# feinanshan/TDNet

Hardware: AMD Instinct MI355X
Metric: frames/sec (td4-psp18, 1024x2048, full-resolution logits) (higher is better)
Workload: dtype f32; 1 GPU; td4-psp18, 1024x2048 Cityscapes-shaped synthetic stream, 3-frame feature cache, 1 clip per GPU; parallelism=clip-parallel x1, RCCL weight broadcast only, target_fps_per_gpu=30

## Files before the change

### tdnet_amd/csrc/td_launch.h

```cpp
#pragma once
#include "td_weights.h"

#ifdef TDNET_TIMING_PROBES
static int probe_skip() {
    static const int m = [] {
        const char* e = getenv("TDNET_PROBE_SKIP");
        const int v = e ? atoi(e) : 0;
        if (v) fprintf(stderr, "tdnet: TDNET_PROBE_SKIP=%d -- pieces of the frame are NOT computed, every result of this process is garbage (timing probe build)\n", v);
        return v;
    }();
    return m;
}
#else
static constexpr int probe_skip() { return 0; }
#endif
static void prof_begin(tdnet* n, int family, int dominant, double flops, hipStream_t s) {
    if (!n || !n->prof) return;
    if (n->nrec == n->recs.size()) {
        ProfRec r;
        hipEventCreate(&r.e0); hipEventCreate(&r.e1);
        n->recs.push_back(r);
    }
    ProfRec& r = n->recs[n->nrec];
    r.family = family; r.dominant = dominant; r.flops = flops;
    hipEventRecord(r.e0, s);
}
static void prof_end(tdnet* n, hipStream_t s) {
    if (!n || !n->prof) return;
    hipEventRecord(n->recs[n->nrec].e1, s);
    n->nrec++;
}

struct LnFuse { const float *mean, *rstd, *g, *b; };

struct WinoChunk { int ny = 1, cy = 0, nx = 1, cx = 0; };

template <int VW>
static void launch_wino4_c(bool out_side, const WinoArgs& wa, hipStream_t s) {
    if (out_side) TD_LAUNCH((k_wino4_out_c<VW>), dim3(wino_chunk_grid(wa.Tc, wa.Cout, VW)), dim3(256), 0, s, wa);
    else TD_LAUNCH((k_wino4_in_c<VW>), dim3(wino_chunk_grid(wa.Tc, wa.C, VW)), dim3(256), 0, s, wa);
}

static ConvArgs conv_args(const ConvLayer& L, const float* in, int H, int W, const float* resid, float* out) {
    const int Ho = out_size(H, L.KS, L.stride, L.dil, L.pad), Wo = out_size(W, L.KS, L.stride, L.dil, L.pad);
    return ConvArgs{in, L.d_wp, L.d_bias, resid, out, H, W, L.Cin, Wo, L.Cout, L.CoutPad, L.stride, L.dil, L.pad, Ho * Wo, L.nsteps, L.act, 0, 1};
}
static GemmArgs gemm_args(const ConvLayer& L, const float* a, int M, int nbatch, const float* bias, const float* resid, float* out, int act) {
    GemmArgs ga;
    ga.a = a; ga.wp = L.d_wp; ga.bias = bias; ga.resid = resid; ga.out = out;
    ga.M = M; ga.N = L.Cout; ga.NPad = L.CoutPad; ga.K = L.Cin; ga.nbatch = nbatch; ga.act = act; ga.tiles_m = ga.tiles_n = 0; ga.MP = M;
    return ga;
}
static void launch_gemm(const ConvLayer& L, const GemmArgs& ga, int b3_grid, hipStream_t s) {
    const int forced_grid = L.pers > 1 ? L.pers : 0;
    switch (L.gemm) {
    case GK_B3: gemm_b3_launch(ga, forced_grid ? forced_grid : b3_grid, s); break;
    case GK_DMA: gemm_dma_launch(ga, forced_grid, s); break;
    case GK_PERSISTENT: gemm_launch(ga, L.tile, forced_grid, s); break;
    case GK_CONV:
        conv_launch(ConvArgs{ga.a, ga.wp, ga.bias, ga.resid, ga.out, 1, ga.M, ga.K, ga.M, ga.N, ga.NPad, 1, 1, 0, ga.M, L.nsteps, ga.act, 0, ga.nbatch}, L.tile, 1, false, s);
        break;
    }
}

static int run_wino(tdnet* n, const ConvLayer& L, const float* in, int H, int W, const float* resid, float* out, hipStream_t s,
                    const LnFuse* lnf, const WinoChunk& ck, float* V, float* Mb, const ClsArgs* cls = nullptr) {
    const int TY = wino_tiles_1d(H, L.dil, L.wino), TX = wino_tiles_1d(W, L.dil, L.wino);
    const long T = (long)L.dil * L.dil * TY * TX;
    const bool chunked = ck.ny != 1 || ck.nx != 1;
    if (chunked && (!L.vw || L.dil % ck.ny || L.dil % ck.nx)) return td_fail("internal: this conv cannot run in chunks");
    const long Tc = (long)(L.dil / ck.ny) * (L.dil / ck.nx) * TY * TX;
    const int nb = (L.wino + 2) * (L.wino + 2);
    bool own = false;
    if (!V) {
        own = n == nullptr || n->wino_v_floats < (size_t)nb * Tc * L.Cin || n->wino_m_floats < (size_t)nb * Tc * L.Cout;
        if (own) {
            if (n) { n->failed = true; return td_fail("internal: Winograd workspace too small"); }
            if (dev_alloc(&V, (size_t)nb * Tc * L.Cin) || dev_alloc(&Mb, (size_t)nb * Tc * L.Cout)) return -1;
        } else { V = n->wino_v; Mb = n->wino_m; }
    }
    WinoArgs wa;
    wa.in = in; wa.V = V; wa.Mb = Mb; wa.bias = L.d_bias; wa.resid = resid; wa.out = out;
    wa.H = H; wa.W = W; wa.C = L.Cin; wa.Cout = L.Cout; wa.dil = L.dil; wa.TY = TY; wa.TX = TX; wa.T = (int)T; wa.act = L.act; wa.TP = (int)Tc;
    wa.ln_mean = lnf ? lnf->mean : nullptr; wa.ln_rstd = lnf ? lnf->rstd : nullptr; wa.ln_g = lnf ? lnf->g : nullptr; wa.ln_b = lnf ? lnf->b : nullptr;
    wa.Tc = (int)Tc; wa.ny = ck.ny; wa.cy = ck.cy; wa.nx = ck.nx; wa.cx = ck.cx;
    auto transform = [&](bool out_side) {
        if (n && (probe_skip() & 1)) return;
        prof_begin(n, 2, false, 0, s);
        const int C = out_side ? L.Cout : L.Cin;
        if (out_side && cls) {
            const unsigned grid = (unsigned)((Tc + 3) / 4);
            if (L.Cout == 128) TD_LAUNCH((k_wino4_out_cls<2>), dim3(grid), dim3(256), wino_out_cls_lds(128, cls->NC), s, wa, *cls);
            else TD_LAUNCH((k_wino4_out_cls<1>), dim3(grid), dim3(256), wino_out_cls_lds(64, cls->NC), s, wa, *cls);
        } else
        if (L.vw == 1) launch_wino4_c<1>(out_side, wa, s);
        else if (L.vw == 2 && C % 2 == 0) launch_wino4_c<2>(out_side, wa, s);
        else if (L.vw == 4 && C % 4 == 0) launch_wino4_c<4>(out_side, wa, s);
        else if (L.vw) launch_wino4_c<1>(out_side, wa, s);
        else if (out_side) TD_LAUNCH(k_wino4_out, dim3(td_grid_for(T * (L.Cout / 4), 256, 256 * 16)), dim3(256), 0, s, wa);
        else TD_LAUNCH(k_wino4_in, dim3(td_grid_for(T * (L.Cin / 4), 256, 256 * 16)), dim3(256), 0, s, wa);
        prof_end(n, s);
    };
    transform(false);
    prof_begin(n, 0, 2, 2.0 * nb * Tc * (double)L.Cin * L.Cout, s);
    if (!(n && (probe_skip() & 8))) launch_gemm(L, gemm_args(L, V, (int)Tc, nb, L.d_zero, nullptr, Mb, 0), chunked ? 320 : 0, s);
    prof_end(n, s);
    transform(true);
    if (own) { TD_HIP(hipStreamSynchronize(s)); hipFree(V); hipFree(Mb); }
    return 0;
}

static void launch_conv_dma_forms(const ConvLayer& L, const ConvArgs& a, hipStream_t s) {
    int rh = L.rh;
    bool done = false;
    const bool is192 = rh == CD_192_P || rh == CD_192_N;
    if (rh == CD_128_N || rh == CD_192_N) {
        done = !L.rowimg_off && conv_launch_dma3n(a, rh, L.KS, L.out16, s);
        if (!done) rh = is192 ? CD_192_P : CD_128_P;
    }
    if (!done && (rh == CD_128_P || rh == CD_192_P)) {
        done = !L.rowimg_off && conv_launch_dma3p(a, rh, L.KS, L.out16, s);
        if (!done) rh = is192 ? CD_192 : CD_128_8W;
    }
    if (!done && (L.rowimg_off || !conv_launch_dma3(a, rh, L.KS, L.out16, s))) conv_launch_dma(a, rh, L.KS, L.out16, s);
}

static int run_conv(tdnet* n, const ConvLayer& L, const float* in, int H, int W, const float* resid, float* out, hipStream_t s,
                    int* Ho_out = nullptr, int* Wo_out = nullptr, const LnFuse* lnf = nullptr, const ClsArgs* cls = nullptr) {
    if (lnf && !L.wino) return td_fail("internal: LayerNorm fusion needs a Winograd input transform");
    if (cls && (!L.wino || L.chunks > 1 || resid)) return td_fail("internal: the classifier rides in a whole Winograd conv's output transform");
    const int Ho = out_size(H, L.KS, L.stride, L.dil, L.pad), Wo = out_size(W, L.KS, L.stride, L.dil, L.pad);
    if (L.wino) {
        if (Ho_out) *Ho_out = H;
        if (Wo_out) *Wo_out = W;
        if (L.chunks > 1 && (!n || !n->ws_ready)) {
            for (int c = 0; c < L.chunks; ++c) {
                WinoChunk ck; ck.ny = L.chunks; ck.cy = c;
                TD_TRY(run_wino(n, L, in, H, W, resid, out, s, lnf, ck, nullptr, nullptr));
            }
            return 0;
        }
        return run_wino(n, L, in, H, W, resid, out, s, lnf, WinoChunk(), nullptr, nullptr, cls);
    }
    const ConvArgs a = conv_args(L, in, H, W, resid, out);
    prof_begin(n, 0, (((L.tile == CT_128x128 || L.tile == CT_128x128_DEEP || L.rh) && L.KS == 3 && !L.stem) ? 1 : 0) | ((L.h16() && L.in16 && L.KS == 3 && !L.stem) ? 4 : 0), L.flops_per_pixel() * a.M, s);
    switch (L.route) {
    case CR_STEM_H: conv_launch_stem_h(a, L.out16, s); break;
    case CR_CONV_DMA: launch_conv_dma_forms(L, a, s); break;
    case CR_CONV_H: conv_launch_h(a, L.tile, L.KS, L.in16, L.out16, s); break;
    case CR_ADIRECT_B3: conv_launch_adirect_b3(a, L.KS, 0, s); break;
    case CR_GEMM1X1: launch_gemm(L, gemm_args(L, in, a.M, 1, L.d_bias, resid, out, L.act), 0, s); break;
    case CR_ADIRECT_ROWS:
    case CR_ADIRECT_ROWS_B3: {
        ConvArgs r = a;
        r.H = stem_rows_hp(H); r.W = stem_rows_wp(W); r.Cin = 3; r.pad = 0;
        if (L.route == CR_ADIRECT_ROWS_B3) conv_launch_adirect_b3(r, L.KS, 2, s);
        else conv_launch_adirect(r, L.KS, 2, s);
        break;
    }
    case CR_ADIRECT: conv_launch_adirect(a, L.KS, L.stem ? 1 : 0, s); break;
    case CR_IGEMM: conv_launch(a, L.tile, L.KS, L.stem, s); break;
    case CR_WINO: break;
    }
    prof_end(n, s);
    if (Ho_out) *Ho_out = Ho;
    if (Wo_out) *Wo_out = Wo;
    return 0;
}

struct ConvCall { const ConvLayer* L; const float* in; int H, W; float* out; };
static int run_conv_group(tdnet* n, const ConvCall* c, int ng, hipStream_t s, int* Ho_out = nullptr, int* Wo_out = nullptr) {
    bool same = n && (n->opts.fusion & TDNET_FUSION_CONV_GROUPS) && ng >= 2 && ng <= 3;
    for (int g = 0; same && g < ng; ++g) {
        const ConvLayer& L = *c[g].L;
        const ConvLayer& L0 = *c[0].L;
        same = L.route == CR_CONV_H && L.in16 == L.out16 && L.in16 == L0.in16 && (g == 0 ? (L.KS == 1 || L.KS == 3) : L.KS == 1) &&
               conv_tile_dims(L.tile).BM == conv_tile_dims(L0.tile).BM && conv_tile_dims(L.tile).BN == conv_tile_dims(L0.tile).BN;
    }
    if (!same) {
        for (int g = 0; g < ng; ++g) TD_TRY(run_conv(n, *c[g].L, c[g].in, c[g].H, c[g].W, nullptr, c[g].out, s, g == 0 ? Ho_out : nullptr, g == 0 ? Wo_out : nullptr));
        return 0;
    }
    ConvArgs a[3];
// ... 99 lines not shown
```

### tdnet_amd/csrc/td_wino.h

```cpp
#pragma once
#include "td_conv.h"

#include <vector>

struct WinoArgs {
    const float* in;
    float* V;
    const float* Mb;
    const float* bias;
    const float* resid;
    float* out;
    int H, W, C, Cout, dil, TY, TX, T, act;
    int TP;
    const float* ln_mean; const float* ln_rstd; const float* ln_g; const float* ln_b;
    int Tc, ny, cy, nx, cx;
};
struct WinoBufs { TdBuf in, g, b, resid, out; };
TD_DEV WinoBufs td_wino_bufs(const WinoArgs& p) {
    WinoBufs w;
    const unsigned pix = (unsigned)p.H * (unsigned)p.W;
    w.in = td_make_buf(p.in, pix * (unsigned)p.C * 4u);
    w.g = td_make_buf(p.ln_g, p.ln_mean ? pix * 4u : 0u);
    w.b = td_make_buf(p.ln_b, p.ln_mean ? pix * 4u : 0u);
    w.resid = td_make_buf(p.resid, p.resid ? pix * (unsigned)p.Cout * 4u : 0u);
    w.out = td_make_buf(p.out, pix * (unsigned)p.Cout * 4u);
    return w;
}
TD_DEV f32x4 td_wino_ld(const WinoArgs& p, const WinoBufs& w, int y, int x, int cv, const f32x4& m4, const f32x4& r4) {
    const bool ok = (unsigned)y < (unsigned)p.H && (unsigned)x < (unsigned)p.W;
    const unsigned pix = (unsigned)y * (unsigned)p.W + (unsigned)x;
    f32x4 z = td_buf_ld4(w.in, ok ? (pix * (unsigned)p.C + (unsigned)cv * 4u) * 4u : TD_BUF_OOB, 0u);
    if (p.ln_mean) {
        const float g = td_buf_ld1(w.g, ok ? pix * 4u : TD_BUF_OOB, 0u), b = td_buf_ld1(w.b, ok ? pix * 4u : TD_BUF_OOB, 0u);
        z = (z - m4) * r4 * g + b;
    }
    return z;
}

TD_DEV void td_wino4_bt(const f32x4 (&d)[6], f32x4 (&t)[6]) {
    const f32x4 a = d[4] - 4.f * d[2], b = d[3] - 4.f * d[1], c = d[4] - d[2], e = 2.f * (d[3] - d[1]);
    t[0] = 4.f * d[0] - 5.f * d[2] + d[4];
    t[1] = a + b;
    t[2] = a - b;
    t[3] = c + e;
    t[4] = c - e;
    t[5] = 4.f * d[1] - 5.f * d[3] + d[5];
}
TD_DEV void td_wino4_at(const f32x4 (&m)[6], f32x4 (&y)[4]) {
    const f32x4 p = m[1] + m[2], q = m[1] - m[2], r = m[3] + m[4], s = m[3] - m[4];
    y[0] = m[0] + p + r;
    y[1] = q + 2.f * s;
    y[2] = p + 4.f * r;
    y[3] = q + 8.f * s + m[5];
}

TD_KERNEL void TD_LAUNCH_BOUNDS(256, 2) k_wino4_in(WinoArgs p) {
    const int CV = p.C >> 2;
    const WinoBufs wb = td_wino_bufs(p);
    const long total = (long)p.T * CV;
    for (long i = (long)blockIdx.x * blockDim.x + threadIdx.x; i < total; i += (long)gridDim.x * blockDim.x) {
        const int cv = (int)(i % CV);
        int t = (int)(i / CV);
        const int tx = t % p.TX; t /= p.TX;
        const int ty = t % p.TY; t /= p.TY;
        const int px = t % p.dil, py = t / p.dil;
        f32x4 tm[6][6];
        f32x4 m4 = {0.f, 0.f, 0.f, 0.f}, r4 = m4;
        if (p.ln_mean) { m4 = td_ld4(p.ln_mean + cv * 4); r4 = td_ld4(p.ln_rstd + cv * 4); }
#pragma unroll
        for (int c = 0; c < 6; ++c) {
            const int x = px + p.dil * (4 * tx - 1 + c);
            f32x4 d[6], col[6];
#pragma unroll
            for (int r = 0; r < 6; ++r) d[r] = td_wino_ld(p, wb, py + p.dil * (4 * ty - 1 + r), x, cv, m4, r4);
            td_wino4_bt(d, col);
#pragma unroll
            for (int r = 0; r < 6; ++r) tm[r][c] = col[r];
        }
        const size_t tile = (size_t)(i / CV);
#pragma unroll
        for (int r = 0; r < 6; ++r) {
            f32x4 v[6];
            td_wino4_bt(tm[r], v);
#pragma unroll
            for (int c = 0; c < 6; ++c) td_st4(p.V + ((size_t)(r * 6 + c) * p.TP + tile) * p.C + cv * 4, v[c]);
        }
    }
}

TD_KERNEL void TD_LAUNCH_BOUNDS(256, 2) k_wino4_out(WinoArgs p) {
    const int CV = p.Cout >> 2;
    const WinoBufs wb = td_wino_bufs(p);
    const float slope = td_act_slope(p.act);
    const long total = (long)p.T * CV;
    for (long i = (long)blockIdx.x * blockDim.x + threadIdx.x; i < total; i += (long)gridDim.x * blockDim.x) {
        const int cv = (int)(i % CV);
        const size_t tile = (size_t)(i / CV);
        int t = (int)tile;
        const int tx = t % p.TX; t /= p.TX;
        const int ty = t % p.TY; t /= p.TY;
        const int px = t % p.dil, py = t / p.dil;
        unsigned offy[4], offx[4];
        bool oky[4], okx[4];
#pragma unroll
        for (int r = 0; r < 4; ++r) {
            const int y = py + p.dil * (4 * ty + r), x = px + p.dil * (4 * tx + r);
            oky[r] = y < p.H; okx[r] = x < p.W;
            offy[r] = (unsigned)y * (unsigned)p.W * (unsigned)p.Cout * 4u;
            offx[r] = ((unsigned)x * (unsigned)p.Cout + (unsigned)cv * 4u) * 4u;
        }
        f32x4 rs[4][4];
#pragma unroll
        for (int r = 0; r < 4; ++r)
#pragma unroll
            for (int c = 0; c < 4; ++c) rs[r][c] = td_buf_ld4(wb.resid, (oky[r] && okx[c]) ? offy[r] + offx[c] : TD_BUF_OOB, 0u);
        f32x4 sm[4][6];
#pragma unroll
        for (int c = 0; c < 6; ++c) {
            f32x4 m[6], col[4];
#pragma unroll
            for (int r = 0; r < 6; ++r) m[r] = td_ld4(p.Mb + ((size_t)(r * 6 + c) * p.TP + tile) * p.Cout + cv * 4);
            td_wino4_at(m, col);
#pragma unroll
            for (int r = 0; r < 4; ++r) sm[r][c] = col[r];
        }
        const f32x4 b = td_ld4(p.bias + cv * 4);
#pragma unroll
        for (int r = 0; r < 4; ++r) {
            f32x4 o4[4];
            td_wino4_at(sm[r], o4);
#pragma unroll
            for (int c = 0; c < 4; ++c) {
                f32x4 o = o4[c] + b;
                o = o + rs[r][c];
#pragma unroll
                for (int e = 0; e < 4; ++e) o[e] = td_activate(o[e], slope);
                td_buf_st4(wb.out, (oky[r] && okx[c]) ? offy[r] + offx[c] : TD_BUF_OOB, o);
            }
        }
    }
}


template <int VW> struct WinoVec;
template <> struct WinoVec<1> {
    typedef float T;
    TD_DEV_MEMBER T ld(TdBuf b, unsigned v, unsigned s) { return td_buf_ld1(b, v, s); }
    TD_DEV_MEMBER void st(TdBuf b, unsigned v, unsigned s, T x) { td_buf_st1(b, v, s, x); }
    TD_DEV_MEMBER T act(T x, float slope) { return td_activate(x, slope); }
};
template <> struct WinoVec<2> {
    typedef f32x2 T;
    TD_DEV_MEMBER T ld(TdBuf b, unsigned v, unsigned s) { return td_buf_ld2(b, v, s); }
    TD_DEV_MEMBER void st(TdBuf b, unsigned v, unsigned s, T x) { td_buf_st2(b, v, s, x); }
    TD_DEV_MEMBER T act(T x, float slope) { x[0] = td_activate(x[0], slope); x[1] = td_activate(x[1], slope); return x; }
};
template <> struct WinoVec<4> {
    typedef f32x4 T;
    TD_DEV_MEMBER T ld(TdBuf b, unsigned v, unsigned s) { return td_buf_ld4(b, v == TD_BUF_OOB ? v : v + s, 0u); }
    TD_DEV_MEMBER void st(TdBuf b, unsigned v, unsigned s, T x) { td_buf_st4(b, v == TD_BUF_OOB ? v : v + s, x); }
    TD_DEV_MEMBER T act(T x, float slope) {
#pragma unroll
        for (int e = 0; e < 4; ++e) x[e] = td_activate(x[e], slope);
        return x;
    }
};
template <typename T>
TD_DEV void td_wino4_bt_t(const T (&d)[6], T (&t)[6]) {
    const T a = d[4] - 4.f * d[2], b = d[3] - 4.f * d[1], c = d[4] - d[2], e = 2.f * (d[3] - d[1]);
    t[0] = 4.f * d[0] - 5.f * d[2] + d[4];
    t[1] = a + b;
    t[2] = a - b;
    t[3] = c + e;
    t[4] = c - e;
    t[5] = 4.f * d[1] - 5.f * d[3] + d[5];
}
template <typename T>
TD_DEV void td_wino4_at_t(const T (&m)[6], T (&y)[4]) {
    const T p = m[1] + m[2], q = m[1] - m[2], r = m[3] + m[4], s = m[3] - m[4];
    y[0] = m[0] + p + r;
    y[1] = q + 2.f * s;
    y[2] = p + 4.f * r;
    y[3] = q + 8.f * s + m[5];
}
struct WinoTile { int tl, sl, py, px, ty, tx; };
TD_DEV WinoTile td_wino_unit_tile(const WinoArgs& p, int slices, int wv) {
    WinoTile w;
    w.tl = wv / slices; w.sl = wv - w.tl * slices;
    int t = w.tl;
    w.tx = t % p.TX; t /= p.TX;
    w.ty = t % p.TY; t /= p.TY;
    const int pw = p.dil / p.nx;
    w.px = p.nx * (t % pw) + p.cx;
    w.py = p.ny * (t / pw) + p.cy;
    return w;
}

template <int VW, typename Mid>
TD_DEV void td_wino4_in_unit(const WinoArgs& p, int wv, Mid&& mid) {
    typedef WinoVec<VW> X;
    typedef typename X::T T;
    const int slices = (p.C + 64 * VW - 1) / (64 * VW);
    const WinoTile w = td_wino_unit_tile(p, slices, wv);
    const WinoBufs wb = td_wino_bufs(p);
    const int c0 = (w.sl * 64 + (int)(threadIdx.x & 63)) * VW;
    const unsigned coff = c0 < p.C ? (unsigned)c0 * 4u : TD_BUF_OOB;
    T m4 = T(0.f), r4 = T(0.f);
    if (p.ln_mean) {
        const TdBuf mb = td_make_buf(p.ln_mean, (unsigned)p.C * 4u), rb = td_make_buf(p.ln_rstd, (unsigned)p.C * 4u);
        m4 = X::ld(mb, coff, 0u); r4 = X::ld(rb, coff, 0u);
    }
    T dd[6][6];
#pragma unroll
    for (int c = 0; c < 6; ++c) {
        const int x = w.px + p.dil * (4 * w.tx - 1 + c);
#pragma unroll
        for (int r = 0; r < 6; ++r) {
            const int y = w.py + p.dil * (4 * w.ty - 1 + r);
            const bool ok = (unsigned)y < (unsigned)p.H && (unsigned)x < (unsigned)p.W;
            const unsigned pix = (unsigned)y * (unsigned)p.W + (unsigned)x;
            T z = X::ld(wb.in, ok ? coff : TD_BUF_OOB, ok ? pix * (unsigned)p.C * 4u : 0u);
            if (p.ln_mean) {
                const float g = td_buf_ld1(wb.g, ok ? 0u : TD_BUF_OOB, ok ? pix * 4u : 0u), b = td_buf_ld1(wb.b, ok ? 0u : TD_BUF_OOB, ok ? pix * 4u : 0u);
                z = (z - m4) * r4 * g + b;
            }
            dd[c][r] = z;
        }
    }
    mid();
    T tm[6][6];
#pragma unroll
    for (int c = 0; c < 6; ++c) {
        T col[6];
        td_wino4_bt_t(dd[c], col);
#pragma unroll
        for (int r = 0; r < 6; ++r) tm[r][c] = col[r];
    }
    mid();
    const unsigned plane = (unsigned)p.TP * (unsigned)p.C * 4u;
    const TdBuf vb = td_make_buf(p.V, 36u * plane);
    const unsigned voff = (unsigned)w.tl * (unsigned)p.C * 4u;
#pragma unroll
    for (int r = 0; r < 6; ++r) {
        T v[6];
        td_wino4_bt_t(tm[r], v);
#pragma unroll
        for (int c = 0; c < 6; ++c) X::st(vb, coff, (unsigned)(r * 6 + c) * plane + voff, v[c]);
    }
}

template <int VW, typename Mid>
TD_DEV void td_wino4_out_unit(const WinoArgs& p, int wv, Mid&& mid) {
    typedef WinoVec<VW> X;
    typedef typename X::T T;
    const int slices = (p.Cout + 64 * VW - 1) / (64 * VW);
    const WinoTile w = td_wino_unit_tile(p, slices, wv);
    const WinoBufs wb = td_wino_bufs(p);
    const float slope = td_act_slope(p.act);
    const int c0 = (w.sl * 64 + (int)(threadIdx.x & 63)) * VW;
    const unsigned coff = c0 < p.Cout ? (unsigned)c0 * 4u : TD_BUF_OOB;
    unsigned offy[4], offx[4];
    bool oky[4], okx[4];
#pragma unroll
    for (int r = 0; r < 4; ++r) {
        const int y = w.py + p.dil * (4 * w.ty + r), x = w.px + p.dil * (4 * w.tx + r);
        oky[r] = y < p.H; okx[r] = x < p.W;
        offy[r] = (unsigned)y * (unsigned)p.W * (unsigned)p.Cout * 4u;
        offx[r] = (unsigned)x * (unsigned)p.Cout * 4u;
    }
    T rs[4][4];
#pragma unroll
    for (int r = 0; r < 4; ++r)
#pragma unroll
        for (int c = 0; c < 4; ++c) {
            const bool ok = oky[r] && okx[c];
            rs[r][c] = X::ld(wb.resid, ok ? coff : TD_BUF_OOB, ok ? offy[r] + offx[c] : 0u);
        }
    const unsigned plane = (unsigned)p.TP * (unsigned)p.Cout * 4u;
    const TdBuf mb = td_make_buf(p.Mb, 36u * plane);
    const unsigned moff = (unsigned)w.tl * (unsigned)p.Cout * 4u;
    T mm[6][6];
#pragma unroll
    for (int c = 0; c < 6; ++c)
#pragma unroll
        for (int r = 0; r < 6; ++r) mm[c][r] = X::ld(mb, coff, (unsigned)(r * 6 + c) * plane + moff);
    const TdBuf bbuf = td_make_buf(p.bias, (unsigned)p.Cout * 4u);
    const T b = X::ld(bbuf, coff, 0u);
    mid();
    T sm[4][6];
#pragma unroll
    for (int c = 0; c < 6; ++c) {
        T col[4];
        td_wino4_at_t(mm[c], col);
#pragma unroll
        for (int r = 0; r < 4; ++r) sm[r][c] = col[r];
    }
    mid();
#pragma unroll
    for (int r = 0; r < 4; ++r) {
        T o4[4];
        td_wino4_at_t(sm[r], o4);
#pragma unroll
        for (int c = 0; c < 4; ++c) {
            const bool ok = oky[r] && okx[c];
            T o = o4[c] + b;
            o = o + rs[r][c];
            X::st(wb.out, ok ? coff : TD_BUF_OOB, ok ? offy[r] + offx[c] : 0u, X::act(o, slope));
        }
    }
}

template <int VW>
TD_KERNEL void TD_LAUNCH_BOUNDS(256, VW == 4 ? 2 : 4) k_wino4_in_c(WinoArgs p) {
    const int slices = (p.C + 64 * VW - 1) / (64 * VW);
    const int wv = TD_UNIFORM((int)((blockIdx.x * blockDim.x + threadIdx.x) >> 6));
    if (wv >= p.Tc * slices) return;
    td_wino4_in_unit<VW>(p, wv, []() {});
}
template <int VW>
TD_KERNEL void TD_LAUNCH_BOUNDS(256, VW == 4 ? 2 : 4) k_wino4_out_c(WinoArgs p) {
    const int slices = (p.Cout + 64 * VW - 1) / (64 * VW);
    const int wv = TD_UNIFORM((int)((blockIdx.x * blockDim.x + threadIdx.x) >> 6));
    if (wv >= p.Tc * slices) return;
    td_wino4_out_unit<VW>(p, wv, []() {});
}
struct ClsArgs { const float* w; const float* b; float* out; int NC; };
template <int VW>
TD_KERNEL void TD_LAUNCH_BOUNDS(256, 2) k_wino4_out_cls(WinoArgs p, ClsArgs c) {
    typedef WinoVec<VW> X;
    typedef typename X::T T;
    constexpr int C = 64 * VW, ROW = C + 4;
    TD_DYN_LDS(smem);
    float* ws = reinterpret_cast<float*>(smem);
    float* ys = ws + c.NC * C + (threadIdx.x >> 6) * (16 * ROW);
    for (int i = threadIdx.x; i < c.NC * C; i += blockDim.x) ws[i] = c.w[i];
    __syncthreads();
    const int wv = TD_UNIFORM((int)((blockIdx.x * blockDim.x + threadIdx.x) >> 6));
    if (wv >= p.Tc) return;
    const int lane = threadIdx.x & 63;
    const WinoTile w = td_wino_unit_tile(p, 1, wv);
    const float slope = td_act_slope(p.act);
    const unsigned coff = (unsigned)(lane * VW) * 4u;
    const unsigned plane = (unsigned)p.TP * (unsigned)C * 4u;
    const TdBuf mb = td_make_buf(p.Mb, 36u * plane);
    const unsigned moff = (unsigned)w.tl * (unsigned)C * 4u;
    T mm[6][6];
#pragma unroll
    for (int cc = 0; cc < 6; ++cc)
#pragma unroll
        for (int r = 0; r < 6; ++r) mm[cc][r] = X::ld(mb, coff, (unsigned)(r * 6 + cc) * plane + moff);
    const TdBuf bbuf = td_make_buf(p.bias, (unsigned)C * 4u);
    const T b = X::ld(bbuf, coff, 0u);
    T sm[4][6];
#pragma unroll
    for (int cc = 0; cc < 6; ++cc) {
        T col[4];
        td_wino4_at_t(mm[cc], col);
#pragma unroll
        for (int r = 0; r < 4; ++r) sm[r][cc] = col[r];
    }
#pragma unroll
    for (int r = 0; r < 4; ++r) {
        T o4[4];
        td_wino4_at_t(sm[r], o4);
#pragma unroll
        for (int cc = 0; cc < 4; ++cc) {
            T o = o4[cc] + b;
            o = o + T(0.f);
            o = X::act(o, slope);
            float* dst = ys + (r * 4 + cc) * ROW + lane * VW;
            if constexpr (VW == 1) dst[0] = o;
            else { dst[0] = o[0]; dst[1] = o[1]; }
        }
    }
    td_wave_sync();
    const int CQ = C >> 2;
    for (int idx = lane; idx < 16 * c.NC; idx += 64) {
        const int px = idx & 15, k = idx >> 4;
        const float* yr = ys + px * ROW;
        const float* wr = ws + k * C;
        float s[4];
#pragma unroll
        for (int qd = 0; qd < 4; ++qd) {
            float a = 0.f;
            for (int ch = 0; ch < CQ; ch += 4) {
                const f32x4 v = td_ld4(yr + qd * CQ + ch), u = td_ld4(wr + qd * CQ + ch);
                a = fmaf(v[0], u[0], a); a = fmaf(v[1], u[1], a); a = fmaf(v[2], u[2], a); a = fmaf(v[3], u[3], a);
            }
            s[qd] = a;
        }
        const int y = w.py + p.dil * (4 * w.ty + (px >> 2)), x = w.px + p.dil * (4 * w.tx + (px & 3));
        if (y < p.H && x < p.W) c.out[(size_t)k * p.H * p.W + (size_t)y * p.W + x] = (((s[0] + s[1]) + s[2]) + s[3]) + c.b[k];
    }
}
static inline bool wino_out_cls_supports(int Cout, int NC) { return (Cout == 64 || Cout == 128) && NC >= 1 && NC <= 32; }
static inline int wino_out_cls_lds(int Cout, int NC) { return (NC * Cout + 4 * 16 * (Cout + 4)) * 4; }

static inline unsigned wino_chunk_grid(int Tc, int C, int VW) { return (unsigned)(((long)Tc * ((C + 64 * VW - 1) / (64 * VW)) + 3) / 4); }


static inline int wino_tiles_1d(int n, int dil, int m) { return ((n + dil - 1) / dil + m - 1) / m; }
static inline long wino_tiles(int H, int W, int dil, int m) { return (long)dil * dil * wino_tiles_1d(H, dil, m) * wino_tiles_1d(W, dil, m); }

static inline long wino_tiles_estimate(long M, int dil, int m) {
    int H = 1;
    while ((long)H * H * 2 < M) ++H;
    const int W = (int)((M + H - 1) / H);
    return wino_tiles(H, W, dil, m);
}

static inline void wino_transform_weights(const float* w, int Cout, int Cin, int m, std::vector<std::vector<float>>& U) {
    static const double G4[6][3] = {{1.0 / 4, 0, 0}, {-1.0 / 6, -1.0 / 6, -1.0 / 6}, {-1.0 / 6, 1.0 / 6, -1.0 / 6},
                                    {1.0 / 24, 1.0 / 12, 1.0 / 6}, {1.0 / 24, -1.0 / 12, 1.0 / 6}, {0, 0, 1}};
    const int n = m + 2;
    const double (*G)[3] = G4;
    U.assign((size_t)n * n, std::vector<float>((size_t)Cout * Cin));
    for (int co = 0; co < Cout; ++co)
        for (int ci = 0; ci < Cin; ++ci) {
            const float* g = w + ((size_t)co * Cin + ci) * 9;
            double t[6][3];
            for (int i = 0; i < n; ++i)
                for (int j = 0; j < 3; ++j) t[i][j] = G[i][0] * g[0 * 3 + j] + G[i][1] * g[1 * 3 + j] + G[i][2] * g[2 * 3 + j];
            for (int i = 0; i < n; ++i)
                for (int j = 0; j < n; ++j)
                    U[(size_t)i * n + j][(size_t)co * Cin + ci] = (float)(t[i][0] * G[j][0] + t[i][1] * G[j][1] + t[i][2] * G[j][2]);
        }
// ... 2 lines not shown
```

Before: 276.5 frames/s.

## Streamline Winograd transform kernels with packed math, magic division and branchless bounds

Reworks the Winograd input and output transform kernels. Integer division is replaced by precomputed magic-multiply reciprocals, and boundary checks become branchless masks. The arithmetic is written as f32x2 packed FMA operations, with inline v_pk_mul/v_pk_add for the LayerNorm scaling. ReLU-only layers are specialised through a template flag so the general activation path is skipped, and all loads are hoisted ahead of compute, with new size guards added. This aims to cut ALU and address overhead in transform kernels that run over full-resolution maps, at the cost of more register pressure and inline assembly that is tied to the target ISA.

Result: faster. 284.1 frames/s, median of 6 (+2.7%).

```diff
diff --git a/tdnet_amd/csrc/td_launch.h b/tdnet_amd/csrc/td_launch.h
--- a/tdnet_amd/csrc/td_launch.h
+++ b/tdnet_amd/csrc/td_launch.h
@@ -36,8 +36,10 @@
 struct WinoChunk { int ny = 1, cy = 0, nx = 1, cx = 0; };
 
 template <int VW>
-static void launch_wino4_c(bool out_side, const WinoArgs& wa, hipStream_t s) {
-    if (out_side) TD_LAUNCH((k_wino4_out_c<VW>), dim3(wino_chunk_grid(wa.Tc, wa.Cout, VW)), dim3(256), 0, s, wa);
+static void launch_wino4_c(bool out_side, WinoArgs wa, hipStream_t s) {
+    wa.mg_sl = wino_magic(((out_side ? wa.Cout : wa.C) + 64 * VW - 1) / (64 * VW));
+    if (out_side && wino_act_general(wa.act)) TD_LAUNCH((k_wino4_out_c<VW, true>), dim3(wino_chunk_grid(wa.Tc, wa.Cout, VW)), dim3(256), 0, s, wa);
+    else if (out_side) TD_LAUNCH((k_wino4_out_c<VW, false>), dim3(wino_chunk_grid(wa.Tc, wa.Cout, VW)), dim3(256), 0, s, wa);
     else TD_LAUNCH((k_wino4_in_c<VW>), dim3(wino_chunk_grid(wa.Tc, wa.C, VW)), dim3(256), 0, s, wa);
 }
 
@@ -84,6 +86,11 @@
     wa.H = H; wa.W = W; wa.C = L.Cin; wa.Cout = L.Cout; wa.dil = L.dil; wa.TY = TY; wa.TX = TX; wa.T = (int)T; wa.act = L.act; wa.TP = (int)Tc;
     wa.ln_mean = lnf ? lnf->mean : nullptr; wa.ln_rstd = lnf ? lnf->rstd : nullptr; wa.ln_g = lnf ? lnf->g : nullptr; wa.ln_b = lnf ? lnf->b : nullptr;
     wa.Tc = (int)Tc; wa.ny = ck.ny; wa.cy = ck.cy; wa.nx = ck.nx; wa.cx = ck.cx;
+    const long cmax = L.Cin > L.Cout ? L.Cin : L.Cout;
+    if ((long)nb * Tc * cmax * 4 >= (1l << 31) || (long)H * W * cmax * 4 >= (1l << 31) ||
+        (L.vw && !(wino_magic_ok(Tc * ((cmax + 63) / 64), TX) && wino_magic_ok(0, TY) && wino_magic_ok(0, L.dil))))
+        return td_fail("internal: this conv is too large for the Winograd transforms");
+    wa.mg_sl = wino_magic(1); wa.mg_tx = wino_magic(TX); wa.mg_ty = wino_magic(TY); wa.pw = L.dil / ck.nx; wa.mg_pw = wino_magic(wa.pw);
     auto transform = [&](bool out_side) {
         if (n && (probe_skip() & 1)) return;
         prof_begin(n, 2, false, 0, s);
@@ -97,7 +104,8 @@
         else if (L.vw == 2 && C % 2 == 0) launch_wino4_c<2>(out_side, wa, s);
         else if (L.vw == 4 && C % 4 == 0) launch_wino4_c<4>(out_side, wa, s);
         else if (L.vw) launch_wino4_c<1>(out_side, wa, s);
-        else if (out_side) TD_LAUNCH(k_wino4_out, dim3(td_grid_for(T * (L.Cout / 4), 256, 256 * 16)), dim3(256), 0, s, wa);
+        else if (out_side && wino_act_general(wa.act)) TD_LAUNCH((k_wino4_out<true>), dim3(td_grid_for(T * (L.Cout / 4), 256, 256 * 16)), dim3(256), 0, s, wa);
+        else if (out_side) TD_LAUNCH((k_wino4_out<false>), dim3(td_grid_for(T * (L.Cout / 4), 256, 256 * 16)), dim3(256), 0, s, wa);
         else TD_LAUNCH(k_wino4_in, dim3(td_grid_for(T * (L.Cin / 4), 256, 256 * 16)), dim3(256), 0, s, wa);
         prof_end(n, s);
     };
@@ -128,7 +136,7 @@
 static int run_conv(tdnet* n, const ConvLayer& L, const float* in, int H, int W, const float* resid, float* out, hipStream_t s,
                     int* Ho_out = nullptr, int* Wo_out = nullptr, const LnFuse* lnf = nullptr, const ClsArgs* cls = nullptr) {
     if (lnf && !L.wino) return td_fail("internal: LayerNorm fusion needs a Winograd input transform");
-    if (cls && (!L.wino || L.chunks > 1 || resid)) return td_fail("internal: the classifier rides in a whole Winograd conv's output transform");
+    if (cls && (!L.wino || L.chunks > 1 || resid || wino_act_general(L.act))) return td_fail("internal: the classifier rides in a whole Winograd conv's output transform");
     const int Ho = out_size(H, L.KS, L.stride, L.dil, L.pad), Wo = out_size(W, L.KS, L.stride, L.dil, L.pad);
     if (L.wino) {
         if (Ho_out) *Ho_out = H;
diff --git a/tdnet_amd/csrc/td_wino.h b/tdnet_amd/csrc/td_wino.h
--- a/tdnet_amd/csrc/td_wino.h
+++ b/tdnet_amd/csrc/td_wino.h
@@ -14,7 +14,12 @@
     int TP;
     const float* ln_mean; const float* ln_rstd; const float* ln_g; const float* ln_b;
     int Tc, ny, cy, nx, cx;
+    int pw;
+    unsigned long long mg_sl, mg_tx, mg_ty, mg_pw;
 };
+static inline unsigned long long wino_magic(int d) { return (1ull << 40) / (unsigned long long)d + 1ull; }
+static inline bool wino_magic_ok(long n, int d) { return n < (1l << 24) && d > 0 && d < (1 << 16); }
+TD_DEV int td_w_div(int n, unsigned long long m) { return (int)(((unsigned long long)(unsigned)n * m) >> 40); }
 struct WinoBufs { TdBuf in, g, b, resid, out; };
 TD_DEV WinoBufs td_wino_bufs(const WinoArgs& p) {
     WinoBufs w;
@@ -26,208 +31,261 @@
     w.out = td_make_buf(p.out, pix * (unsigned)p.Cout * 4u);
     return w;
 }
-TD_DEV f32x4 td_wino_ld(const WinoArgs& p, const WinoBufs& w, int y, int x, int cv, const f32x4& m4, const f32x4& r4) {
-    const bool ok = (unsigned)y < (unsigned)p.H && (unsigned)x < (unsigned)p.W;
-    const unsigned pix = (unsigned)y * (unsigned)p.W + (unsigned)x;
-    f32x4 z = td_buf_ld4(w.in, ok ? (pix * (unsigned)p.C + (unsigned)cv * 4u) * 4u : TD_BUF_OOB, 0u);
-    if (p.ln_mean) {
-        const float g = td_buf_ld1(w.g, ok ? pix * 4u : TD_BUF_OOB, 0u), b = td_buf_ld1(w.b, ok ? pix * 4u : TD_BUF_OOB, 0u);
-        z = (z - m4) * r4 * g + b;
-    }
-    return z;
-}
-
-TD_DEV void td_wino4_bt(const f32x4 (&d)[6], f32x4 (&t)[6]) {
-    const f32x4 a = d[4] - 4.f * d[2], b = d[3] - 4.f * d[1], c = d[4] - d[2], e = 2.f * (d[3] - d[1]);
-    t[0] = 4.f * d[0] - 5.f * d[2] + d[4];
+struct f32x2p { f32x2 lo, hi; };
+TD_DEV f32x2p operator+(f32x2p a, f32x2p b) { return f32x2p{a.lo + b.lo, a.hi + b.hi}; }
+TD_DEV f32x2p operator-(f32x2p a, f32x2p b) { return f32x2p{a.lo - b.lo, a.hi - b.hi}; }
+TD_DEV f32x2p operator-(f32x2p a) { return f32x2p{-a.lo, -a.hi}; }
+TD_DEV f32x2p td_w_split(f32x4 v) { return f32x2p{f32x2{v[0], v[1]}, f32x2{v[2], v[3]}}; }
+TD_DEV f32x4 td_w_join(f32x2p v) { return f32x4{v.lo[0], v.lo[1], v.hi[0], v.hi[1]}; }
+TD_DEV float td_w_fma(float k, float x, float y) { return __builtin_fmaf(k, x, y); }
+TD_DEV f32x2 td_w_fma(float k, f32x2 x, f32x2 y) { return __builtin_elementwise_fma(f32x2{k, k}, x, y); }
+TD_DEV f32x2p td_w_fma(float k, f32x2p x, f32x2p y) { return f32x2p{td_w_fma(k, x.lo, y.lo), td_w_fma(k, x.hi, y.hi)}; }
+TD_DEV float td_w_mul(float k, float x) { return k * x; }
+TD_DEV f32x2 td_w_mul(float k, f32x2 x) { return k * x; }
+TD_DEV f32x2p td_w_mul(float k, f32x2p x) { return f32x2p{k * x.lo, k * x.hi}; }
+TD_DEV float td_w_ln(float z, float m, float r, float g, float b) { return (z - m) * r * g + b; }
+TD_DEV f32x2 td_w_ln(f32x2 z, f32x2 m, f32x2 r, float g, float b) { return (z - m) * r * g + b; }
+TD_DEV float td_w_ln_u(float z, float m, float r, float g, float b) { return (z - m) * r * g + b; }
+TD_DEV f32x2 td_w_ln_u(f32x2 z, f32x2 m, f32x2 r, float g, float b) {
+#ifdef TD_EMU
+    return (z - m) * r * g + b;
+#else
+    const f32x2 t = (z - m) * r;
+    const unsigned long long gp = __builtin_bit_cast(unsigned, g), bp = __builtin_bit_cast(unsigned, b);
+    f32x2 u, v;
+    asm("v_pk_mul_f32 %0, %1, %2 op_sel_hi:[1,0]" : "=v"(u) : "v"(t), "s"(gp));
+    asm("v_pk_add_f32 %0, %1, %2 op_sel_hi:[1,0]" : "=v"(v) : "v"(u), "s"(bp));
+    return v;
+#endif
+}
+TD_DEV f32x2p td_w_ln_u(f32x2p z, f32x2p m, f32x2p r, float g, float b) { return f32x2p{td_w_ln_u(z.lo, m.lo, r.lo, g, b), td_w_ln_u(z.hi, m.hi, r.hi, g, b)}; }
+TD_DEV f32x2p td_w_ln(f32x2p z, f32x2p m, f32x2p r, float g, float b) { return f32x2p{td_w_ln(z.lo, m.lo, r.lo, g, b), td_w_ln(z.hi, m.hi, r.hi, g, b)}; }
+
+template <typename T>
+TD_DEV void td_wino4_bt_t(const T (&d)[6], T (&t)[6]) {
+    const T a = td_w_fma(-4.f, d[2], d[4]), b = td_w_fma(-4.f, d[1], d[3]);
+    const T c = d[4] - d[2], x = d[3] - d[1];
+    t[0] = td_w_fma(4.f, d[0], -td_w_mul(5.f, d[2])) + d[4];
     t[1] = a + b;
     t[2] = a - b;
-    t[3] = c + e;
-    t[4] = c - e;
-    t[5] = 4.f * d[1] - 5.f * d[3] + d[5];
-}
-TD_DEV void td_wino4_at(const f32x4 (&m)[6], f32x4 (&y)[4]) {
-    const f32x4 p = m[1] + m[2], q = m[1] - m[2], r = m[3] + m[4], s = m[3] - m[4];
+    t[3] = td_w_fma(2.f, x, c);
+    t[4] = td_w_fma(-2.f, x, c);
+    t[5] = td_w_fma(4.f, d[1], -td_w_mul(5.f, d[3])) + d[5];
+}
+template <typename T>
+TD_DEV void td_wino4_at_t(const T (&m)[6], T (&y)[4]) {
+    const T p = m[1] + m[2], q = m[1] - m[2], r = m[3] + m[4], s = m[3] - m[4];
     y[0] = m[0] + p + r;
-    y[1] = q + 2.f * s;
-    y[2] = p + 4.f * r;
-    y[3] = q + 8.f * s + m[5];
-}
+    y[1] = td_w_fma(2.f, s, q);
+    y[2] = td_w_fma(4.f, r, p);
+    y[3] = td_w_fma(8.f, s, q) + m[5];
+}
+
+TD_DEV float td_w_relu(float v) { return __builtin_elementwise_maximum(v, -0.f); }
+template <bool GEN> TD_DEV float td_w_act(float v, float slope) { return GEN ? td_activate(v, slope) : td_w_relu(v); }
+template <bool GEN> TD_DEV f32x2 td_w_act(f32x2 v, float slope) { return f32x2{td_w_act<GEN>(v[0], slope), td_w_act<GEN>(v[1], slope)}; }
+template <bool GEN> TD_DEV f32x2p td_w_act(f32x2p v, float slope) { return f32x2p{td_w_act<GEN>(v.lo, slope), td_w_act<GEN>(v.hi, slope)}; }
+template <bool GEN, typename T, int N>
+TD_DEV void td_wino_activate(T (&o)[N], int act) {
+    if (GEN || act == 1) {
+        const float slope = td_act_slope(act);
+#pragma unroll
+        for (int i = 0; i < N; ++i) o[i] = td_w_act<GEN>(o[i], slope);
+    }
+}
+TD_HOSTDEV bool wino_act_general(int act) { return act == 2; }
 
 TD_KERNEL void TD_LAUNCH_BOUNDS(256, 2) k_wino4_in(WinoArgs p) {
     const int CV = p.C >> 2;
     const WinoBufs wb = td_wino_bufs(p);
+    const unsigned plane = (unsigned)p.TP * (unsigned)p.C * 4u;
+    const TdBuf vb = td_make_buf(p.V, 36u * plane);
     const long total = (long)p.T * CV;
     for (long i = (long)blockIdx.x * blockDim.x + threadIdx.x; i < total; i += (long)gridDim.x * blockDim.x) {
         const int cv = (int)(i % CV);
-        int t = (int)(i / CV);
+        const unsigned tile = (unsigned)(i / CV);
+        int t = (int)tile;
         const int tx = t % p.TX; t /= p.TX;
         const int ty = t % p.TY; t /= p.TY;
         const int px = t % p.dil, py = t / p.dil;
-        f32x4 tm[6][6];
-        f32x4 m4 = {0.f, 0.f, 0.f, 0.f}, r4 = m4;
-        if (p.ln_mean) { m4 = td_ld4(p.ln_mean + cv * 4); r4 = td_ld4(p.ln_rstd + cv * 4); }
+        unsigned offy[6], offx[6], piy[6], pix[6];
+#pragma unroll
+        for (int r = 0; r < 6; ++r) {
+            const int y = py + p.dil * (4 * ty - 1 + r), x = px + p.dil * (4 * tx - 1 + r);
+            const bool oky = (unsigned)y < (unsigned)p.H, okx = (unsigned)x < (unsigned)p.W;
+            piy[r] = oky ? (unsigned)y * (unsigned)p.W * 4u : TD_BUF_OOB;
+            pix[r] = okx ? (unsigned)x * 4u : TD_BUF_OOB;
+            offy[r] = oky ? (unsigned)y * (unsigned)p.W * (unsigned)p.C * 4u : TD_BUF_OOB;
+            offx[r] = okx ? ((unsigned)x * (unsigned)p.C + (unsigned)cv * 4u) * 4u : TD_BUF_OOB;
+        }
+        f32x2p dd[6][6];
+#pragma unroll
+        for (int c = 0; c < 6; ++c)
+#pragma unroll
+            for (int r = 0; r < 6; ++r) dd[c][r] = td_w_split(td_buf_ld4(wb.in, __builtin_elementwise_add_sat(offy[r], offx[c]), 0u));
+        if (p.ln_mean) {
+            const f32x2p m4 = td_w_split(td_ld4(p.ln_mean + cv * 4)), r4 = td_w_split(td_ld4(p.ln_rstd + cv * 4));
+#pragma unroll
+            for (int c = 0; c < 6; ++c)
+#pragma unroll
+                for (int r = 0; r < 6; ++r) {
+                    const unsigned po = __builtin_elementwise_add_sat(piy[r], pix[c]);
+                    dd[c][r] = td_w_ln(dd[c][r], m4, r4, td_buf_ld1(wb.g, po, 0u), td_buf_ld1(wb.b, po, 0u));
+                }
+        }
+        f32x2p tm[6][6];
 #pragma unroll
         for (int c = 0; c < 6; ++c) {
-            const int x = px + p.dil * (4 * tx - 1 + c);
-            f32x4 d[6], col[6];
-#pragma unroll
-            for (int r = 0; r < 6; ++r) d[r] = td_wino_ld(p, wb, py + p.dil * (4 * ty - 1 + r), x, cv, m4, r4);
-            td_wino4_bt(d, col);
+            f32x2p col[6];
+            td_wino4_bt_t(dd[c], col);
 #pragma unroll
             for (int r = 0; r < 6; ++r) tm[r][c] = col[r];
         }
-        const size_t tile = (size_t)(i / CV);
+        const unsigned voff = (tile * (unsigned)p.C + (unsigned)cv * 4u) * 4u;
 #pragma unroll
         for (int r = 0; r < 6; ++r) {
-            f32x4 v[6];
-            td_wino4_bt(tm[r], v);
-#pragma unroll
-            for (int c = 0; c < 6; ++c) td_st4(p.V + ((size_t)(r * 6 + c) * p.TP + tile) * p.C + cv * 4, v[c]);
-        }
-    }
-}
-
+            f32x2p v[6];
+            td_wino4_bt_t(tm[r], v);
+#pragma unroll
+            for (int c = 0; c < 6; ++c) td_buf_st4(vb, voff + (unsigned)(r * 6 + c) * plane, td_w_join(v[c]));
+        }
+    }
+}
+
+template <bool GEN>
 TD_KERNEL void TD_LAUNCH_BOUNDS(256, 2) k_wino4_out(WinoArgs p) {
     const int CV = p.Cout >> 2;
     const WinoBufs wb = td_wino_bufs(p);
-    const float slope = td_act_slope(p.act);
+    const unsigned plane = (unsigned)p.TP * (unsigned)p.Cout * 4u;
+    const TdBuf mb = td_make_buf(p.Mb, 36u * plane);
     const long total = (long)p.T * CV;
     for (long i = (long)blockIdx.x * blockDim.x + threadIdx.x; i < total; i += (long)gridDim.x * blockDim.x) {
         const int cv = (int)(i % CV);
-        const size_t tile = (size_t)(i / CV);
+        const unsigned tile = (unsigned)(i / CV);
         int t = (int)tile;
         const int tx = t % p.TX; t /= p.TX;
         const int ty = t % p.TY; t /= p.TY;
         const int px = t % p.dil, py = t / p.dil;
         unsigned offy[4], offx[4];
-        bool oky[4], okx[4];
 #pragma unroll
         for (int r = 0; r < 4; ++r) {
             const int y = py + p.dil * (4 * ty + r), x = px + p.dil * (4 * tx + r);
-            oky[r] = y < p.H; okx[r] = x < p.W;
-            offy[r] = (unsigned)y * (unsigned)p.W * (unsigned)p.Cout * 4u;
-            offx[r] = ((unsigned)x * (unsigned)p.Cout + (unsigned)cv * 4u) * 4u;
-        }
-        f32x4 rs[4][4];
+            offy[r] = y < p.H ? (unsigned)y * (unsigned)p.W * (unsigned)p.Cout * 4u : TD_BUF_OOB;
+            offx[r] = x < p.W ? ((unsigned)x * (unsigned)p.Cout + (unsigned)cv * 4u) * 4u : TD_BUF_OOB;
+        }
+        f32x2p o[16];
 #pragma unroll
         for (int r = 0; r < 4; ++r)
 #pragma unroll
-            for (int c = 0; c < 4; ++c) rs[r][c] = td_buf_ld4(wb.resid, (oky[r] && okx[c]) ? offy[r] + offx[c] : TD_BUF_OOB, 0u);
-        f32x4 sm[4][6];
+            for (int c = 0; c < 4; ++c) o[r * 4 + c] = td_w_split(td_buf_ld4(wb.resid, __builtin_elementwise_add_sat(offy[r], offx[c]), 0u));
+        const unsigned moff = (tile * (unsigned)p.Cout + (unsigned)cv * 4u) * 4u;
+        f32x2p mm[6][6];
+#pragma unroll
+        for (int c = 0; c < 6; ++c)
+#pragma unroll
+            for (int r = 0; r < 6; ++r) mm[c][r] = td_w_split(td_buf_ld4(mb, moff, (unsigned)(r * 6 + c) * plane));
+        const f32x2p b = td_w_split(td_ld4(p.bias + cv * 4));
+        f32x2p sm[4][6];
 #pragma unroll
         for (int c = 0; c < 6; ++c) {
-            f32x4 m[6], col[4];
-#pragma unroll
-            for (int r = 0; r < 6; ++r) m[r] = td_ld4(p.Mb + ((size_t)(r * 6 + c) * p.TP + tile) * p.Cout + cv * 4);
-            td_wino4_at(m, col);
+            f32x2p col[4];
+            td_wino4_at_t(mm[c], col);
 #pragma unroll
             for (int r = 0; r < 4; ++r) sm[r][c] = col[r];
         }
-        const f32x4 b = td_ld4(p.bias + cv * 4);
 #pragma unroll
         for (int r = 0; r < 4; ++r) {
-            f32x4 o4[4];
-            td_wino4_at(sm[r], o4);
-#pragma unroll
-            for (int c = 0; c < 4; ++c) {
-                f32x4 o = o4[c] + b;
-                o = o + rs[r][c];
-#pragma unroll
-                for (int e = 0; e < 4; ++e) o[e] = td_activate(o[e], slope);
-                td_buf_st4(wb.out, (oky[r] && okx[c]) ? offy[r] + offx[c] : TD_BUF_OOB, o);
-            }
-        }
-    }
-}
-
-
+            f32x2p o4[4];
+            td_wino4_at_t(sm[r], o4);
+#pragma unroll
+            for (int c = 0; c < 4; ++c) o[r * 4 + c] = (o4[c] + b) + o[r * 4 + c];
+        }
+        td_wino_activate<GEN>(o, p.act);
+#pragma unroll
+        for (int r = 0; r < 4; ++r)
+#pragma unroll
+            for (int c = 0; c < 4; ++c) td_buf_st4(wb.out, __builtin_elementwise_add_sat(offy[r], offx[c]), td_w_join(o[r * 4 + c]));
+    }
+}
+
+
+TD_DEV TdBuf td_wino_row_buf(const float* base, unsigned off_bytes, unsigned bytes) {
+    return td_make_buf(reinterpret_cast<const float*>(reinterpret_cast<const char*>(base) + off_bytes), bytes);
+}
 template <int VW> struct WinoVec;
 template <> struct WinoVec<1> {
     typedef float T;
+    TD_DEV_MEMBER T zero() { return 0.f; }
     TD_DEV_MEMBER T ld(TdBuf b, unsigned v, unsigned s) { return td_buf_ld1(b, v, s); }
-    TD_DEV_MEMBER void st(TdBuf b, unsigned v, unsigned s, T x) { td_buf_st1(b, v, s, x); }
-    TD_DEV_MEMBER T act(T x, float slope) { return td_activate(x, slope); }
+    TD_DEV_MEMBER void st(TdBuf b, unsigned v, T x) { td_buf_st1(b, v, 0u, x); }
 };
 template <> struct WinoVec<2> {
     typedef f32x2 T;
+    TD_DEV_MEMBER T zero() { return f32x2{0.f, 0.f}; }
     TD_DEV_MEMBER T ld(TdBuf b, unsigned v, unsigned s) { return td_buf_ld2(b, v, s); }
-    TD_DEV_MEMBER void st(TdBuf b, unsigned v, unsigned s, T x) { td_buf_st2(b, v, s, x); }
-    TD_DEV_MEMBER T act(T x, float slope) { x[0] = td_activate(x[0], slope); x[1] = td_activate(x[1], slope); return x; }
+    TD_DEV_MEMBER void st(TdBuf b, unsigned v, T x) { td_buf_st2(b, v, 0u, x); }
 };
 template <> struct WinoVec<4> {
-    typedef f32x4 T;
-    TD_DEV_MEMBER T ld(TdBuf b, unsigned v, unsigned s) { return td_buf_ld4(b, v == TD_BUF_OOB ? v : v + s, 0u); }
-    TD_DEV_MEMBER void st(TdBuf b, unsigned v, unsigned s, T x) { td_buf_st4(b, v == TD_BUF_OOB ? v : v + s, x); }
-    TD_DEV_MEMBER T act(T x, float slope) {
-#pragma unroll
-        for (int e = 0; e < 4; ++e) x[e] = td_activate(x[e], slope);
-        return x;
-    }
+    typedef f32x2p T;
+    TD_DEV_MEMBER T zero() { return f32x2p{f32x2{0.f, 0.f}, f32x2{0.f, 0.f}}; }
+    TD_DEV_MEMBER T ld(TdBuf b, unsigned v, unsigned s) { return td_w_split(td_buf_ld4(b, v, s)); }
+    TD_DEV_MEMBER void st(TdBuf b, unsigned v, T x) { td_buf_st4(b, v, td_w_join(x)); }
 };
-template <typename T>
-TD_DEV void td_wino4_bt_t(const T (&d)[6], T (&t)[6]) {
-    const T a = d[4] - 4.f * d[2], b = d[3] - 4.f * d[1], c = d[4] - d[2], e = 2.f * (d[3] - d[1]);
-    t[0] = 4.f * d[0] - 5.f * d[2] + d[4];
-    t[1] = a + b;
-    t[2] = a - b;
-    t[3] = c + e;
-    t[4] = c - e;
-    t[5] = 4.f * d[1] - 5.f * d[3] + d[5];
-}
-template <typename T>
-TD_DEV void td_wino4_at_t(const T (&m)[6], T (&y)[4]) {
-    const T p = m[1] + m[2], q = m[1] - m[2], r = m[3] + m[4], s = m[3] - m[4];
-    y[0] = m[0] + p + r;
-    y[1] = q + 2.f * s;
-    y[2] = p + 4.f * r;
-    y[3] = q + 8.f * s + m[5];
-}
 struct WinoTile { int tl, sl, py, px, ty, tx; };
 TD_DEV WinoTile td_wino_unit_tile(const WinoArgs& p, int slices, int wv) {
     WinoTile w;
-    w.tl = wv / slices; w.sl = wv - w.tl * slices;
-    int t = w.tl;
-    w.tx = t % p.TX; t /= p.TX;
-    w.ty = t % p.TY; t /= p.TY;
-    const int pw = p.dil / p.nx;
-    w.px = p.nx * (t % pw) + p.cx;
-    w.py = p.ny * (t / pw) + p.cy;
+    w.tl = td_w_div(wv, p.mg_sl); w.sl = wv - w.tl * slices;
+    const int t1 = td_w_div(w.tl, p.mg_tx), t2 = td_w_div(t1, p.mg_ty), t3 = td_w_div(t2, p.mg_pw);
+    w.tx = w.tl - t1 * p.TX;
+    w.ty = t1 - t2 * p.TY;
+    w.px = p.nx * (t2 - t3 * p.pw) + p.cx;
+    w.py = p.ny * t3 + p.cy;
     return w;
 }
 
-template <int VW, typename Mid>
-TD_DEV void td_wino4_in_unit(const WinoArgs& p, int wv, Mid&& mid) {
+template <int VW>
+TD_DEV void td_wino4_in_unit(const WinoArgs& p, int wv) {
     typedef WinoVec<VW> X;
     typedef typename X::T T;
     const int slices = (p.C + 64 * VW - 1) / (64 * VW);
     const WinoTile w = td_wino_unit_tile(p, slices, wv);
-    const WinoBufs wb = td_wino_bufs(p);
     const int c0 = (w.sl * 64 + (int)(threadIdx.x & 63)) * VW;
     const unsigned coff = c0 < p.C ? (unsigned)c0 * 4u : TD_BUF_OOB;
-    T m4 = T(0.f), r4 = T(0.f);
+    const unsigned in_bytes = (unsigned)p.H * (unsigned)p.W * (unsigned)p.C * 4u;
+    unsigned sy[6], sx[6], my[6], mx[6], piy[6], pix[6];
+#pragma unroll
+    for (int r = 0; r < 6; ++r) {
+        const int y = w.py + p.dil * (4 * w.ty - 1 + r), x = w.px + p.dil * (4 * w.tx - 1 + r);
+        sy[r] = ((unsigned)y - (unsigned)p.H) & ~(unsigned)y; sx[r] = ((unsigned)x - (unsigned)p.W) & ~(unsigned)x;
+        my[r] = (unsigned)((int)sy[r] >> 31); mx[r] = (unsigned)((int)sx[r] >> 31);
+        piy[r] = (unsigned)y * (unsigned)p.W; pix[r] = (unsigned)x;
+    }
+    T dd[6][6];
+#pragma unroll
+    for (int c = 0; c < 6; ++c)
+#pragma unroll
+        for (int r = 0; r < 6; ++r) {
+            const unsigned ok = my[r] & mx[c];
+            dd[c][r] = X::ld(td_make_buf(p.in, in_bytes & ok), coff, ((piy[r] + pix[c]) & ok) * (unsigned)p.C * 4u);
+        }
     if (p.ln_mean) {
         const TdBuf mb = td_make_buf(p.ln_mean, (unsigned)p.C * 4u), rb = td_make_buf(p.ln_rstd, (unsigned)p.C * 4u);
-        m4 = X::ld(mb, coff, 0u); r4 = X::ld(rb, coff, 0u);
-    }
-    T dd[6][6];
-#pragma unroll
-    for (int c = 0; c < 6; ++c) {
-        const int x = w.px + p.dil * (4 * w.tx - 1 + c);
-#pragma unroll
-        for (int r = 0; r < 6; ++r) {
-            const int y = w.py + p.dil * (4 * w.ty - 1 + r);
-            const bool ok = (unsigned)y < (unsigned)p.H && (unsigned)x < (unsigned)p.W;
-            const unsigned pix = (unsigned)y * (unsigned)p.W + (unsigned)x;
-            T z = X::ld(wb.in, ok ? coff : TD_BUF_OOB, ok ? pix * (unsigned)p.C * 4u : 0u);
-            if (p.ln_mean) {
-                const float g = td_buf_ld1(wb.g, ok ? 0u : TD_BUF_OOB, ok ? pix * 4u : 0u), b = td_buf_ld1(wb.b, ok ? 0u : TD_BUF_OOB, ok ? pix * 4u : 0u);
-                z = (z - m4) * r4 * g + b;
+        const T m4 = X::ld(mb, coff, 0u), r4 = X::ld(rb, coff, 0u);
+        unsigned gy[6], gx[6];
+#pragma unroll
+        for (int r = 0; r < 6; ++r) { gy[r] = piy[r] & my[r]; gx[r] = pix[r] & mx[r]; }
+#pragma unroll
+        for (int c = 0; c < 6; ++c) {
+#pragma unroll
+            for (int r = 0; r < 6; ++r) {
+                const unsigned ok = (unsigned)((int)(sy[r] & sx[c]) >> 31), pi = gy[r] + gx[c];
+                const float g = __builtin_bit_cast(float, __builtin_bit_cast(unsigned, p.ln_g[pi]) & ok);
+                const float b = __builtin_bit_cast(float, __builtin_bit_cast(unsigned, p.ln_b[pi]) & ok);
+                dd[c][r] = td_w_ln_u(dd[c][r], m4, r4, g, b);
             }
-            dd[c][r] = z;
-        }
-    }
-    mid();
+            TD_SCHED_FENCE();
+        }
+    }
     T tm[6][6];
 #pragma unroll
     for (int c = 0; c < 6; ++c) {
@@ -236,45 +294,42 @@
 #pragma unroll
         for (int r = 0; r < 6; ++r) tm[r][c] = col[r];
     }
-    mid();
     const unsigned plane = (unsigned)p.TP * (unsigned)p.C * 4u;
-    const TdBuf vb = td_make_buf(p.V, 36u * plane);
     const unsigned voff = (unsigned)w.tl * (unsigned)p.C * 4u;
 #pragma unroll
     for (int r = 0; r < 6; ++r) {
         T v[6];
+        TD_SCHED_FENCE();
         td_wino4_bt_t(tm[r], v);
 #pragma unroll
-        for (int c = 0; c < 6; ++c) X::st(vb, coff, (unsigned)(r * 6 + c) * plane + voff, v[c]);
-    }
-}
-
-template <int VW, typename Mid>
-TD_DEV void td_wino4_out_unit(const WinoArgs& p, int wv, Mid&& mid) {
+        for (int c = 0; c < 6; ++c) X::st(td_wino_row_buf(p.V, (unsigned)(r * 6 + c) * plane + voff, (unsigned)p.C * 4u), coff, v[c]);
+    }
+}
+
+template <int VW, bool GEN>
+TD_DEV void td_wino4_out_unit(const WinoArgs& p, int wv) {
     typedef WinoVec<VW> X;
     typedef typename X::T T;
     const int slices = (p.Cout + 64 * VW - 1) / (64 * VW);
     const WinoTile w = td_wino_unit_tile(p, slices, wv);
-    const WinoBufs wb = td_wino_bufs(p);
-    const float slope = td_act_slope(p.act);
     const int c0 = (w.sl * 64 + (int)(threadIdx.x & 63)) * VW;
     const unsigned coff = c0 < p.Cout ? (unsigned)c0 * 4u : TD_BUF_OOB;
-    unsigned offy[4], offx[4];
-    bool oky[4], okx[4];
+    const unsigned res_bytes = p.resid ? (unsigned)p.H * (unsigned)p.W * (unsigned)p.Cout * 4u : 0u;
+    unsigned offy[4], offx[4], my[4], mx[4];
 #pragma unroll
     for (int r = 0; r < 4; ++r) {
         const int y = w.py + p.dil * (4 * w.ty + r), x = w.px + p.dil * (4 * w.tx + r);
-        oky[r] = y < p.H; okx[r] = x < p.W;
+        my[r] = (unsigned)((int)((unsigned)y - (unsigned)p.H) >> 31); mx[r] = (unsigned)((int)((unsigned)x - (unsigned)p.W) >> 31);
         offy[r] = (unsigned)y * (unsigned)p.W * (unsigned)p.Cout * 4u;
         offx[r] = (unsigned)x * (unsigned)p.Cout * 4u;
     }
-    T rs[4][4];
+    T o[16];
 #pragma unroll
     for (int r = 0; r < 4; ++r)
 #pragma unroll
         for (int c = 0; c < 4; ++c) {
-            const bool ok = oky[r] && okx[c];
-            rs[r][c] = X::ld(wb.resid, ok ? coff : TD_BUF_OOB, ok ? offy[r] + offx[c] : 0u);
+            const unsigned ok = my[r] & mx[c];
+            o[r * 4 + c] = X::ld(td_make_buf(p.resid, res_bytes & ok), coff, (offy[r] + offx[c]) & ok);
         }
     const unsigned plane = (unsigned)p.TP * (unsigned)p.Cout * 4u;
     const TdBuf mb = td_make_buf(p.Mb, 36u * plane);
@@ -286,7 +341,6 @@
         for (int r = 0; r < 6; ++r) mm[c][r] = X::ld(mb, coff, (unsigned)(r * 6 + c) * plane + moff);
     const TdBuf bbuf = td_make_buf(p.bias, (unsigned)p.Cout * 4u);
     const T b = X::ld(bbuf, coff, 0u);
-    mid();
     T sm[4][6];
 #pragma unroll
     for (int c = 0; c < 6; ++c) {
@@ -295,19 +349,21 @@
 #pragma unroll
         for (int r = 0; r < 4; ++r) sm[r][c] = col[r];
     }
-    mid();
 #pragma unroll
     for (int r = 0; r < 4; ++r) {
         T o4[4];
         td_wino4_at_t(sm[r], o4);
 #pragma unroll
+        for (int c = 0; c < 4; ++c) o[r * 4 + c] = (o4[c] + b) + o[r * 4 + c];
+    }
+    td_wino_activate<GEN>(o, p.act);
+#pragma unroll
+    for (int r = 0; r < 4; ++r)
+#pragma unroll
         for (int c = 0; c < 4; ++c) {
-            const bool ok = oky[r] && okx[c];
-            T o = o4[c] + b;
-            o = o + rs[r][c];
-            X::st(wb.out, ok ? coff : TD_BUF_OOB, ok ? offy[r] + offx[c] : 0u, X::act(o, slope));
-        }
-    }
+            const unsigned ok = my[r] & mx[c];
+            X::st(td_wino_row_buf(p.out, (offy[r] + offx[c]) & ok, ((unsigned)p.Cout * 4u) & ok), coff, o[r * 4 + c]);
+        }
 }
 
 template <int VW>
@@ -315,14 +371,14 @@
     const int slices = (p.C + 64 * VW - 1) / (64 * VW);
     const int wv = TD_UNIFORM((int)((blockIdx.x * blockDim.x + threadIdx.x) >> 6));
     if (wv >= p.Tc * slices) return;
-    td_wino4_in_unit<VW>(p, wv, []() {});
-}
-template <int VW>
+    td_wino4_in_unit<VW>(p, wv);
+}
+template <int VW, bool GEN>
 TD_KERNEL void TD_LAUNCH_BOUNDS(256, VW == 4 ? 2 : 4) k_wino4_out_c(WinoArgs p) {
     const int slices = (p.Cout + 64 * VW - 1) / (64 * VW);
     const int wv = TD_UNIFORM((int)((blockIdx.x * blockDim.x + threadIdx.x) >> 6));
     if (wv >= p.Tc * slices) return;
-    td_wino4_out_unit<VW>(p, wv, []() {});
+    td_wino4_out_unit<VW, GEN>(p, wv);
 }
 struct ClsArgs { const float* w; const float* b; float* out; int NC; };
 template <int VW>
@@ -339,7 +395,6 @@
     if (wv >= p.Tc) return;
     const int lane = threadIdx.x & 63;
     const WinoTile w = td_wino_unit_tile(p, 1, wv);
-    const float slope = td_act_slope(p.act);
     const unsigned coff = (unsigned)(lane * VW) * 4u;
     const unsigned plane = (unsigned)p.TP * (unsigned)C * 4u;
     const TdBuf mb = td_make_buf(p.Mb, 36u * plane);
@@ -359,19 +414,20 @@
 #pragma unroll
         for (int r = 0; r < 4; ++r) sm[r][cc] = col[r];
     }
+    T o[16];
 #pragma unroll
     for (int r = 0; r < 4; ++r) {
         T o4[4];
         td_wino4_at_t(sm[r], o4);
 #pragma unroll
-        for (int cc = 0; cc < 4; ++cc) {
-            T o = o4[cc] + b;
-            o = o + T(0.f);
-            o = X::act(o, slope);
-            float* dst = ys + (r * 4 + cc) * ROW + lane * VW;
-            if constexpr (VW == 1) dst[0] = o;
-            else { dst[0] = o[0]; dst[1] = o[1]; }
-        }
+        for (int cc = 0; cc < 4; ++cc) o[r * 4 + cc] = (o4[cc] + b) + X::zero();
+    }
+    td_wino_activate<false>(o, p.act);
+#pragma unroll
+    for (int i = 0; i < 16; ++i) {
+        float* dst = ys + i * ROW + lane * VW;
+        if constexpr (VW == 1) dst[0] = o[i];
+        else { dst[0] = o[i][0]; dst[1] = o[i][1]; }
     }
     td_wave_sync();
     const int CQ = C >> 2;
```
